# AlbrechtL/welle.io

Hardware: AMD Instinct MI355X
Metric: DAB Mode-I ensembles/s (x real-time) (higher is better)
Workload: dtype f32 (FFT/demap) + u16 (Viterbi metrics) + u8 (GF(256))

## Files before the change

welle.io_amd/capi.py:

```python
import ctypes as C
import os
import numpy as np

HERE = os.path.dirname(os.path.abspath(__file__))
DEFAULT_LIB = os.path.join(HERE, "libdabphy_hip.so")

T_U, T_S, FRAME_SYMS_LEN = 2048, 2552, 2048 + 75 * 2552
ABI_VERSION = 6


class Config(C.Structure):
    _fields_ = [("struct_size", C.c_uint32), ("n_ensembles", C.c_uint32), ("max_frames", C.c_uint32), ("device", C.c_int32),
                ("fft_placement", C.c_int32), ("disable_coarse", C.c_int32), ("want_constellation", C.c_int32),
                ("want_impulse_response", C.c_int32), ("demod_chunk", C.c_int32), ("freqsync_method", C.c_int32), ("pipeline_sync", C.c_int32), ("serial_sync", C.c_int32), ("no_batch_replay", C.c_int32), ("decode_shape", C.c_int32), ("sync_early", C.c_int32)]


class WidebandConfig(C.Structure):
    _fields_ = [("struct_size", C.c_uint32), ("decimation", C.c_uint32), ("n_taps", C.c_uint32), ("taps", C.POINTER(C.c_float)),
                ("offset_16khz", C.POINTER(C.c_int32)), ("format", C.c_int32)]


class ResamplerConfig(C.Structure):
    _fields_ = [("struct_size", C.c_uint32), ("interpolation", C.c_uint32), ("decimation", C.c_uint32), ("n_taps", C.c_uint32),
                ("taps", C.POINTER(C.c_float)), ("offset_16khz", C.POINTER(C.c_int32)), ("format", C.c_int32)]
# ... 248 lines not shown
        self._chk(self.lib.dabphy_time_viterbi(self.h, nbits, n_codewords, iters, C.byref(a), C.byref(b)))
        return a.value, b.value

    def time_copy(self, nbytes=2 << 30, blocks_per_cu=0, iters=5):
        a = C.c_float(0)
        self._chk(self.lib.dabphy_time_copy(self.h, C.c_uint64(nbytes), blocks_per_cu, iters, C.byref(a)))
        return a.value

    def traceback_split(self, on=True):
        self._chk(self.lib.dabphy_test_traceback_split(self.h, int(on)))

    def last_decode_plan(self):
        a = C.c_int32(0); b = C.c_int32(0)
        self._chk(self.lib.dabphy_last_decode_plan(self.h, C.byref(a), C.byref(b)))
        return a.value, b.value

    def time_fused_msc(self, iters=3):
        a = C.c_float(0)
        self._chk(self.lib.dabphy_time_fused_msc(self.h, iters, C.byref(a)))
        return a.value

    def reset(self):
        self._chk(self.lib.dabphy_reset(self.h))

    def stream_upload(self, iq, loop=False):
        iq = np.ascontiguousarray(iq, np.complex64).reshape(self.cfg.n_ensembles, -1)
        self._chk(self.lib.dabphy_stream_upload(self.h, _p(iq), C.c_uint64(iq.shape[1]), int(loop)))

    def stream_bind_device(self, dev_ptr, ring_samples, stride_samples, n_valid, loop=False):
        self._chk(self.lib.dabphy_stream_bind_device(self.h, C.c_void_p(dev_ptr), C.c_uint64(ring_samples), C.c_uint64(stride_samples),
# ... 352 lines not shown
```

welle.io_amd/csrc/dabphy_api.hip:

```cpp
#include "dabphy_internal.h"
#include <cstddef>

extern "C" {

uint32_t dabphy_abi_version(void) { return DABPHY_ABI_VERSION; }
size_t dabphy_struct_size(int32_t which)
{
    switch (which) {
        case DABPHY_STRUCT_CONFIG: return sizeof(dabphy_config);
        case DABPHY_STRUCT_FRAME_INFO: return sizeof(dabphy_frame_info);
        case DABPHY_STRUCT_SF_EVENT: return sizeof(dabphy_sf_event);
        case DABPHY_STRUCT_SUBCHANNEL: return sizeof(dabphy_subchannel);
        case DABPHY_STRUCT_PROTECTION: return sizeof(dabphy_protection);
        case DABPHY_STRUCT_TII_MEASUREMENT: return sizeof(dabphy_tii_measurement);
        case DABPHY_STRUCT_MSC_DESC: return sizeof(dabphy_msc_desc);
        case DABPHY_STRUCT_MP2_EVENT: return sizeof(dabphy_mp2_event);
        case DABPHY_STRUCT_AU_SERVICE: return sizeof(dabphy_au_service);
        case DABPHY_STRUCT_AU_DESC: return sizeof(dabphy_au_desc);
        case DABPHY_STRUCT_WIDEBAND_CONFIG: return sizeof(dabphy_wideband_config);
        case DABPHY_STRUCT_RESAMPLER_CONFIG: return sizeof(dabphy_resampler_config);
    }
    return 0;
}

// ... 22 lines not shown
    if (cfg_in->struct_size <= offsetof(dabphy_config, freqsync_method)) cfg_full.freqsync_method = 2;
    cfg_full.struct_size = (uint32_t)sizeof(dabphy_config);
    const dabphy_config* const cfg = &cfg_full;
    if (cfg->n_ensembles < 1 || cfg->max_frames < 1) return DABPHY_ERR_INVALID;
    if (cfg->max_frames > DABPHY_MAX_FRAMES || (uint64_t)cfg->n_ensembles * cfg->max_frames > DABPHY_MAX_ENSEMBLE_FRAMES) return DABPHY_ERR_INVALID;
    *out = nullptr;
    int ndev = 0;
    if (hipGetDeviceCount(&ndev) != hipSuccess || ndev <= 0 || cfg->device < 0 || cfg->device >= ndev) return DABPHY_ERR_NO_DEVICE;
    hipDeviceProp_t prop;
    if (hipGetDeviceProperties(&prop, cfg->device) != hipSuccess) return DABPHY_ERR_NO_DEVICE;
    if (strncmp(prop.gcnArchName, "gfx950", 6) != 0) return DABPHY_ERR_NO_DEVICE;
    if (hipSetDevice(cfg->device) != hipSuccess) return DABPHY_ERR_NO_DEVICE;
    dabphy_handle* h = new dabphy_handle();
    h->cfg = *cfg;
    h->subch_e.resize(cfg->n_ensembles); h->subch_next.resize(cfg->n_ensembles); h->where.resize(cfg->n_ensembles); h->kind_next.resize(cfg->n_ensembles);
    if (h->cfg.demod_chunk <= 0) h->cfg.demod_chunk = ((int64_t)h->cfg.n_ensembles * h->cfg.max_frames >= 1024) ? 25 : 15;
    if (h->cfg.demod_chunk > 75) h->cfg.demod_chunk = 75;
    snprintf(h->devname, sizeof h->devname, "%s (%s)", prop.name, prop.gcnArchName);
    int r = 0;
    auto fail = [&](int code) { dabphy_destroy(h); return code; };
    if (h->cfg.fft_placement < 0 || h->cfg.fft_placement > 2 || h->cfg.freqsync_method < 0 || h->cfg.freqsync_method > 2 || h->cfg.pipeline_sync < 0 || h->cfg.pipeline_sync > 3 || h->cfg.decode_shape < 0 || h->cfg.decode_shape > 3 || h->cfg.sync_early < 0 || h->cfg.sync_early > 3) return fail(DABPHY_ERR_INVALID);
    const HostTables& T = host_tables();
    if ((r = upload_const(h, &h->d_tw, T.tw))) return fail(r);
    if ((r = upload_const(h, &h->d_ref, T.ref))) return fail(r);
    if ((r = upload_const(h, &h->d_nco, T.nco))) return fail(r);
    if ((r = upload_const(h, &h->d_bin2soft, T.bin2soft))) return fail(r);
    if ((r = upload_const(h, &h->d_prbs_words, T.prbs_words))) return fail(r);
    dabphy_protection pf; protection_fic(&pf);
    if ((r = upload_const(h, &h->d_fic_map, depuncture_map(&pf)))) return fail(r);
    if ((r = upload_const(h, &h->d_osc_unsafe, T.osc_unsafe))) return fail(r);
    h->tab.tw = h->d_tw; h->tab.ref = h->d_ref; h->tab.nco = h->d_nco; h->tab.bin2soft = h->d_bin2soft; h->tab.prbs_bytes = nullptr;
    h->tab.osc_unsafe = h->d_osc_unsafe; h->tab.n_osc_unsafe = T.n_osc_unsafe;
    if ((r = device_block(h, &h->d_osc_stats, 2, true))) return fail(r);
    if ((r = device_block(h, &h->d_state, cfg->n_ensembles, true))) return fail(r);
    if ((r = device_block(h, &h->d_dec, cfg->n_ensembles, true))) return fail(r);
    {
        int n_placeholders = 5;
#ifdef DABPHY_EXPERIMENTS
        if (const char* e = getenv("DABPHY_STREAM_LAYOUT")) { h->stream_layout = atoi(e); n_placeholders = (h->stream_layout & 1) ? 5 : 0; }
#endif
        hipStream_t placeholder = nullptr;
        for (int i = 0; i < n_placeholders; i++) if ((r = new_stream(h, &placeholder, i == 1))) return fail(r);
    }
    if ((r = new_stream(h, &h->stream))) return fail(r);
    if ((r = new_stream(h, &h->sync_stream, true))) return fail(r);
    if ((r = new_stream(h, &h->aux_stream))) return fail(r);
    if ((r = new_stream(h, &h->copy_stream))) return fail(r);
    if (h->stream_layout & 2) h->fic_stream = h->aux_stream;
// ... 122 lines not shown
    if ((r = ensure(h, h->prs_mag, (size_t)n_frames * T_U * sizeof(float)))) return r;
    if ((r = ensure(h, h->snr, n_frames * sizeof(float)))) return r;
    if (constellation && (r = ensure(h, h->con, (size_t)n_frames * 1200 * sizeof(cf32)))) return r;
    std::vector<FrameDesc> d(n_frames);
    for (uint32_t f = 0; f < n_frames; f++) {
        memset(&d[f], 0, sizeof(FrameDesc));
        d[f].pos = (int64_t)(per * f); d[f].frame_no = f; d[f].valid = 1;
    }
    HIPCHK(h, hipMemcpyAsync(h->iq.p, frames, per * n_frames * sizeof(cf32), hipMemcpyHostToDevice, h->stream));
    HIPCHK(h, hipMemcpyAsync(h->desc.p, d.data(), n_frames * sizeof(FrameDesc), hipMemcpyHostToDevice, h->stream));
    DemodArgs a{};
    a.tab = h->tab; a.iq = h->iq.as<cf32>(); a.iq_stride = 0; a.ring = (int64_t)(per * n_frames);
    a.desc = h->desc.as<FrameDesc>(); a.n_frames = (int)n_frames; a.chunk_len = h->cfg.demod_chunk; a.mix = 0;
    a.soft = h->soft.as<int8_t>(); a.soft_ring = (int)n_frames;
    a.con = constellation ? h->con.as<cf32>() : nullptr; a.prs_mag = h->prs_mag.as<float>();
    launch_demod(a, 1, h->stream);
    SnrArgs s{}; s.state = h->d_dec; s.desc = a.desc; s.n_ens = 1; s.n_frames = (int)n_frames; s.prs_mag = a.prs_mag; s.snr_out = h->snr.as<float>();
    launch_snr(s, h->stream);
    HIPCHK(h, hipMemcpyAsync(soft, h->soft.p, (size_t)n_frames * SOFT_PER_FRAME, hipMemcpyDeviceToHost, h->stream));
    if (constellation) HIPCHK(h, hipMemcpyAsync(constellation, h->con.p, (size_t)n_frames * 1200 * sizeof(cf32), hipMemcpyDeviceToHost, h->stream));
    if (snr) HIPCHK(h, hipMemcpyAsync(snr, h->snr.p, n_frames * sizeof(float), hipMemcpyDeviceToHost, h->stream));
    return sync(h);
}

static int run_lin_decode(dabphy_handle* h, const int8_t* in, size_t in_stride, const map_t* d_map, int nbits, uint32_t n_cw,
                          int dedisperse, uint8_t* out)
{
    int r;
    if ((r = ensure(h, h->in8, in_stride * n_cw))) return r;
    VitClass c{};
    if ((r = prepare_class(h, c, nbits, (int)n_cw, dedisperse))) return r;
// ... 296 lines not shown
    for (uint32_t b = 0; b < n_ens; b++)
        for (uint32_t f = 0; f < n_frames; f++) {
            FrameDesc& x = d[(size_t)b * n_frames + f];
            memset(&x, 0, sizeof x);
            x.pos = (int64_t)(per * f); x.frame_no = f; x.valid = 1; x.f_prs = x.f_sym = f_hz; x.L0 = 12345; x.L1 = 54321;
            const HostTables& T = host_tables();
            for (int i = 0; i < T.n_osc_unsafe; i++) osc_hazard_entry(x.osc_hazard, T.osc_unsafe[i], x.start_index, x.L0, x.f_prs, x.L1, x.f_sym);
        }
    HIPCHK(h, hipMemcpyAsync(h->desc.p, d.data(), total * sizeof(FrameDesc), hipMemcpyHostToDevice, h->stream));
    DemodArgs a{};
    a.tab = h->tab; a.iq = h->iq.as<cf32>(); a.iq_stride = per * n_frames; a.ring = (int64_t)(per * n_frames);
    a.desc = h->desc.as<FrameDesc>(); a.n_frames = (int)n_frames; a.chunk_len = h->cfg.demod_chunk; a.mix = mix;
    a.soft = h->soft.as<int8_t>(); a.soft_ring = (int)n_frames; a.con = nullptr; a.prs_mag = nullptr;
    ScopedEvent e0, e1;
    HIPCHK(h, e0.create()); HIPCHK(h, e1.create());
    launch_demod(a, (int)n_ens, h->stream);
    HIPCHK(h, hipEventRecord(e0, h->stream));
    for (uint32_t i = 0; i < iters; i++) launch_demod(a, (int)n_ens, h->stream);
    HIPCHK(h, hipEventRecord(e1, h->stream));
    HIPCHK(h, hipEventSynchronize(e1));
    float t = 0; HIPCHK(h, hipEventElapsedTime(&t, e0, e1));
    *ms = t / iters;
    return sync(h);
}

int dabphy_time_copy(dabphy_handle* h, uint64_t bytes, uint32_t blocks_per_cu, uint32_t iters, float* gbytes_per_s)
{
    DeviceBind dev_(h);
    if (!h || !gbytes_per_s || bytes < 4096 || iters == 0) return DABPHY_ERR_INVALID;
    hipDeviceProp_t p;
    HIPCHK(h, hipGetDeviceProperties(&p, h->cfg.device));
    const int blocks = p.multiProcessorCount * (int)(blocks_per_cu ? blocks_per_cu : 4);
    DevBuf src, dst; int r;
// ... 43 lines not shown
        float a = 0, b = 0; HIPCHK(h, hipEventElapsedTime(&a, e0, e1)); HIPCHK(h, hipEventElapsedTime(&b, e1, e2));
        tg += a; tv += b;
    }
    *ms_gather = tg / iters; *ms_decode = tv / iters;
    return sync(h);
}

int dabphy_test_traceback_split(dabphy_handle* h, int32_t on)
{
    if (!h) return DABPHY_ERR_INVALID;
    h->tb_split = (on & 1) != 0;
    h->tb_no_walkers = (on & 2) == 0;
    return DABPHY_OK;
}

int dabphy_time_fused_msc(dabphy_handle* h, uint32_t iters, float* ms)
{
    DeviceBind dev_(h);
    if (!h || !ms || iters == 0) return DABPHY_ERR_INVALID;
    const auto& P = h->fplan;
    if (!P.valid || !P.launched || P.buf_gen != h->buf_gen || P.args.n_work == 0) { h->err = "no batch has been decoded by the fused kernel with the present buffers"; return DABPHY_ERR_STATE; }
    HIPCHK(h, hipDeviceSynchronize());
    ScopedEvent e0, e1;
    HIPCHK(h, e0.create()); HIPCHK(h, e1.create());
    const FusedSplit sp{h->tb_no_walkers ? nullptr : h->tb_stream, h->ev_tb_fork, h->ev_tb_join};
    auto again = [&]() { if (P.use_sp) launch_sp(P.args, P.sp_two, P.sp_variant, h->stream); else launch_viterbi_fused(P.args, P.variant, P.n_slots, h->stream, P.args.done ? &sp : nullptr); };
    again();
    HIPCHK(h, hipEventRecord(e0, h->stream));
    for (uint32_t i = 0; i < iters; i++) { again(); if (P.args.done) HIPCHK(h, hipStreamSynchronize(h->stream)); }
    HIPCHK(h, hipEventRecord(e1, h->stream));
// ... 8 lines not shown
```

welle.io_amd/csrc/dabphy_internal.h:

```cpp
#pragma once
#define DABPHY_BUILDING_LIBRARY
#include "../../include/dabphy.h"
#include "../../include/dabphy_test.h"
#include "dabphy_kernels.h"
#include "dabphy_host.h"
#include "osc_exact.h"
#include <string>
#include <vector>
#include <cstring>
#include <cstdio>
#include <cstdlib>
#include <cmath>
#include <algorithm>
#include <chrono>
#include <functional>
#include <numeric>

#define DABPHY_INTERNAL __attribute__((visibility("hidden")))

namespace dabphy {

inline bool debug_env(const char* name)
{
#ifdef DABPHY_EXPERIMENTS
// ... 20 lines not shown
constexpr int SF_BATCH_CLASSES = 256;
constexpr size_t SF_BATCH_BYTES = 3 * (SF_BATCH_CLASSES * sizeof(SfArgs) + (SF_BATCH_CLASSES + 1) * sizeof(int32_t) + 12);
struct HostTimeline { double acc[6] = {0, 0, 0, 0, 0, 0}; long n = 0; };
}
using namespace dabphy;

struct dabphy_handle {
    dabphy_config cfg{};
    hipStream_t stream = nullptr;
    std::string err;
    char devname[256] = {0};
    cf32 *d_tw = nullptr, *d_ref = nullptr, *d_nco = nullptr;
    int16_t* d_bin2soft = nullptr; uint32_t* d_prbs_words = nullptr; map_t* d_fic_map = nullptr;
    int32_t* d_osc_unsafe = nullptr; unsigned long long* d_osc_stats = nullptr;
    Tables tab{};
    DevBuf iq, soft, con, prs_mag, snr, desc, in8, map, vsym, vdec, vout, ok;
    DevBuf fsym, fdec;
    RxState* d_state = nullptr;
    DecState* d_dec = nullptr;
    std::vector<DevBuf> owned;
    std::vector<hipStream_t> streams; std::vector<hipEvent_t> events; std::vector<void*> pinned;

    struct MscClass {
        dabphy_protection prot{};
        std::vector<MscPair> pairs;
        std::vector<int32_t> subch_id, start_cu;
        bool cif0_pending = false;
        DevBuf map, pair_tab, tiles, out;
        DevBuf steps[FUSED_VARIANTS]; int n_windows[FUSED_VARIANTS] = {0, 0, 0};
        DevBuf sf_state;
// ... 261 lines not shown
    ta.tab = h->tab; ta.iq = iq; ta.iq_stride = iq_stride; ta.ring = ring; ta.desc = desc; ta.n_ens = (int)B; ta.n_frames = (int)F;
    ta.rot = h->tii_rot.as<cf32>(); ta.rank = h->tii_rank.as<int32_t>(); ta.pattern = h->tii_pat.as<uint8_t>();
    ta.abs_err = h->tii_err.as<float>(); ta.likely = h->tii_likely.as<int32_t>(); ta.state = h->tii_state.as<TiiSlot>();
    ta.events = h->tii_events.as<TiiEvent>(); ta.n_events = h->tii_nev.as<int32_t>(); ta.max_events = (int)h->tii_max_events;
    ta.overflow = tii_dropped(h);
    return ta;
}

inline int sync(dabphy_handle* h)
{
    HIPCHK(h, hipStreamSynchronize(h->stream));
    HIPCHK(h, hipGetLastError());
    return 0;
}

inline int prepare_class(dabphy_handle* h, VitClass& c, int nbits, int n_cw, int dedisperse)
{
    c.nbits = nbits; c.nsteps = nbits + 6; c.n_cw = n_cw; c.n_groups = (n_cw + 63) / 64; c.dedisperse = dedisperse; c.g_begin = 0; c.g_end = c.n_groups;
    const size_t cells = (size_t)c.n_groups * c.nsteps * 64;
    int r;
    if ((r = ensure(h, h->vsym, cells * sizeof(uint32_t)))) return r;
    if ((r = ensure(h, h->vdec, cells * sizeof(uint2)))) return r;
    if ((r = ensure(h, h->vout, (size_t)c.n_groups * 64 * (nbits / 8)))) return r;
    c.sym = h->vsym.as<uint32_t>(); c.dec = h->vdec.as<uint2>(); c.out = h->vout.as<uint8_t>();
    return 0;
}
inline VitArgs vit_args(const dabphy_handle* h, const VitClass& c) { VitArgs v{}; v.c = c; v.prbs_words = h->d_prbs_words; return v; }
inline FusedClass fic_fused_class(const dabphy_handle* h, uint8_t* out, int n_cw, int variant)
{
    FusedClass fc{}; fc.map = h->d_fic_map; fc.out = out; fc.nbits = 768; fc.nsteps = 774; fc.n_cw = n_cw; fc.n_pairs = 1; fc.kind = 1; fc.dedisperse = 1;
// ... 39 lines not shown
```

welle.io_amd/csrc/dabphy_kernels.h:

```cpp
#pragma once
#include "dabphy_common.h"

namespace dabphy {

struct RxState {
    int64_t pos;
    int64_t frame_no;
    int32_t local_phase;
    int32_t coarse;
    int32_t fine;
    int32_t synced;
    float s_level;
    int32_t lost;
    int32_t n_exact_sums;
    int32_t hist_count, hist_head;
    int32_t hist_dropped;
    int32_t n_relock_inexact;
    int32_t attempts;
    int32_t first_lock_attempts;
    int32_t n_wide_frames;
    int32_t n_chain_frames;
    int32_t calm_frames;
    int32_t acq_phase;
    int32_t acq_counter, acq_idx, acq_left;
// ... 45 lines not shown
    int skip_wide;
    int last_round;
};

struct DemodArgs {
    Tables tab;
    const cf32* iq; size_t iq_stride; int64_t ring;
    const FrameDesc* desc; int n_frames;
    int chunk_len;
    int mix;
    int8_t* soft; int soft_ring;
    size_t soft_ens_stride;
    cf32* con;
    float* prs_mag;
    unsigned long long* osc_stats;
    int frame_first, frame_count, chunk_count;
};

struct SnrArgs {
    DecState* state; const FrameDesc* desc; int n_ens, n_frames;
    const float* prs_mag; float* snr_out;
};

struct VitClass {
    int nbits;
    int nsteps;
    int n_cw;
    int n_groups;
    int g_begin, g_end;
    uint32_t* sym;
    uint2* dec;
// ... 241 lines not shown
struct AuSvc { int32_t n_superframes, n_aus, n_failed; uint32_t bytes; };
struct AuArgs {
    const SfEvent* events; const int32_t* n_events; int n_cif;
    const uint8_t* sf; int n_slots, sf_len;
    const int32_t* run;
    const MscPair* pairs; const int32_t* ens_base;
    int format;
    uint8_t* stage; uint64_t region0, reserve;
    AuSvc* svc; AuRec* aus; uint2* au_src; int au_cap;
};
void launch_au_pack(const AuArgs& a, int n_blocks, hipStream_t s);
void launch_superframe_bucket(const SfBatch& Bt, int bucket, int total_blocks, int n_cif, bool wide_pass, hipStream_t s);
void launch_rs_superframes(const RsArgs& a, hipStream_t s);
void launch_rs_msc(const RsMscArgs& a, hipStream_t s);

void launch_demod(const DemodArgs& a, int n_ens, hipStream_t s);
void launch_snr(const SnrArgs& a, hipStream_t s);
void launch_selftest_div127(unsigned long long* out, hipStream_t s);
void launch_selftest_unit_twiddle(unsigned long long* out, hipStream_t s);
void launch_viterbi(const VitArgs& a, hipStream_t s);
void launch_fic_gather(const FicGatherArgs& a, hipStream_t s);
void launch_msc_gather(const MscGatherArgs& a, hipStream_t s);
void launch_lin_gather(const LinGatherArgs& a, hipStream_t s);
void launch_fib_crc(const CrcArgs& a, hipStream_t s);
void launch_fic_ratio(const CrcArgs& a, hipStream_t s);
#ifdef SYNC_CHAIN_TS
void dump_chain_ts();
#endif
void launch_sync_find(const SyncArgs& a, hipStream_t s);
void launch_sync_wide(const SyncArgs& a, hipStream_t s, hipEvent_t front = nullptr);
void launch_sync_finish(const SyncArgs& a, hipStream_t s);
// ... 6 lines not shown
```

welle.io_amd/csrc/dabphy_process.hip:

```cpp
#include "dabphy_internal.h"

static inline double now_us() { return std::chrono::duration<double, std::micro>(std::chrono::steady_clock::now().time_since_epoch()).count(); }

struct Batch {
    uint32_t B = 0, F = 0;
    int cur = 0, depth = 0;
    int ring_frames = 0; size_t ens_stride = 0;
    FrameDesc* d_desc = nullptr;
    DemodArgs da{};
    VitClass fic{};
    double t0 = 0.0, t[6] = {0, 0, 0, 0, 0, 0};
};

static void tick(const dabphy_handle* h, Batch& b, int i) { if (h->tl_on) b.t[i] = now_us() - b.t0; }
static void mark(dabphy_handle* h, int stage, bool end, hipStream_t st = nullptr)
{
    if (!h->profiling) return;
    hipError_t e = hipEventRecord(end ? h->ev_end[stage] : h->ev_beg[stage], st ? st : h->stream); (void)e;
    h->ev_used[stage] = true;
}

static VitClass fic_class(const dabphy_handle* h, int n_cw)
{
    VitClass c{};
// ... 108 lines not shown
static int replay_fic_frames(dabphy_handle* h, const Batch& b)
{
    const uint32_t B = b.B, F = b.F;
    int r;
    SyncArgs sa = sync_args(h, b.cur, F, h->chain_valid[b.cur]);
    const VitClass c = fic_class(h, (int)(B * 4));
    CrcArgs k = crc_args(h, b);
    FicOneClass fic;
    if ((r = fic_one_prepare(h, fic, fic_gather_args(h, b, c), h->stream))) return r;
    for (uint32_t f = 0; f < F; f++) {
        sa.frame = (int)f;
        launch_sync_find(sa, h->stream);
        launch_sync_finish(sa, h->stream);
        DemodArgs d1 = b.da; d1.frame_first = (int)f; d1.frame_count = 1; d1.con = nullptr; d1.osc_stats = nullptr;
        d1.chunk_count = (3 + b.da.chunk_len - 1) / b.da.chunk_len;
        launch_demod(d1, (int)B, h->stream);
        k.frame_sel = (int)f + 1;
        fic_one_launch(h, fic, (int)f + 1, h->stream);
        launch_fib_crc(k, h->stream);
        CrcArgs kf = k; kf.frame_sel = 0; kf.frame_first = (int)f; kf.frame_count = 1;
        launch_fic_ratio(kf, h->stream);
    }
    return 0;
}

static int queue_next_chains(dabphy_handle* h, const Batch& b)
{
    int r;
    if (h->cfg.pipeline_sync != 2) HIPCHK(h, hipStreamWaitEvent(h->sync_stream, h->ev_chain_gate, 0));
    if (b.depth == 2 && h->ahead < 1 + b.depth && (r = sf_wait_for_pass(h, h->sync_stream))) return r;
    for (; h->ahead < 1 + b.depth; h->ahead++) if ((r = queue_chain(h, (b.cur + h->ahead) % dabphy_handle::N_DESC, b.F))) return r;
// ... 77 lines not shown
        g.map = cls.map.as<map_t>(); g.pairs = cls.pair_tab.as<MscPair>(); g.tiles = cls.tiles.as<int32_t>(); g.n_pairs = P; g.desc = b.d_desc; g.c = c;
        if (first_two) mark(h, dabphy_handle::ST_MSC_GATHER, false);
        launch_msc_gather(g, h->stream);
        launch_viterbi(vit_args(h, c), h->stream);
        first_two = false;
    }
    if (!first_two) mark(h, dabphy_handle::ST_MSC_GATHER, true);
    return 0;
}

static int decode_batch(dabphy_handle* h, Batch& b, const bool replay)
{
    int r;
    if (replay && (r = replay_fic_frames(h, b))) return r;
    mark(h, dabphy_handle::ST_DEMOD, false);
    launch_demod(b.da, (int)b.B, h->stream);
    tick(h, b, 2);
    mark(h, dabphy_handle::ST_DEMOD, true);
    if (!replay && (h->cfg.pipeline_sync == 1 || h->cfg.pipeline_sync == 3)) HIPCHK(h, hipEventRecord(h->ev_chain_gate, h->stream));
    if (!replay && b.depth == 2 && (r = sf_launch_waiting(h))) return r;
    const bool early = h->chain_early || (h->cfg.pipeline_sync != 2 && (h->cfg.sync_early == 0 || h->cfg.sync_early == 3 || (h->cfg.sync_early == 2 && h->drift_seen)));
    if (!replay && b.depth && early) {
        h->wide_front_recorded = false;
        if ((r = queue_next_chains(h, b))) return r;
        if (h->cfg.sync_early == 3 && h->wide_front_recorded) HIPCHK(h, hipStreamWaitEvent(h->stream, h->ev_wide_front, 0));
    }
    if (!replay && (r = sf_launch_waiting(h))) return r;
    if ((r = sf_wait_for_pass(h, h->stream))) return r;
    if ((r = queue_aux_work(h, b))) return r;
    for (auto& cls : h->classes) if (cls.cif0_pending) launch_pair_cif0(cls.pair_tab.as<MscPair>(), (int)cls.pairs.size(), b.d_desc, (int)b.F, h->stream);
    if ((r = launch_fused(h, b))) return r;
// ... 108 lines not shown
```

welle.io_amd/csrc/k_demod.hip:

```cpp
#include "fft2048.h"
#include "dabphy_kernels.h"
#include <dabphy_wave_ops.h>
#include "osc_exact.h"

namespace dabphy {

__device__ __forceinline__ int32_t mod_rate(int64_t x)
{
    int64_t r = x % INPUT_RATE;
    if (r < 0) r += INPUT_RATE;
    return (int32_t)r;
}

struct SymCursor { uint32_t a; int32_t ph; };
struct MixSteps { int32_t s128, sTS; uint32_t s256_bytes; int32_t f1; };

constexpr uint32_t NCO_BYTES = (uint32_t)INPUT_RATE * 8u;

struct OscChain { dc64 base, d128, d256, d512, d1024; };

__device__ __forceinline__ void osc_chain_steps(OscChain& k, int32_t f_hz)
{
    const dc64 a = osc_step(128, f_hz), b = osc_step(256, f_hz), b2 = osc_step(512, f_hz), b4 = osc_step(1024, f_hz);
    k.d128.re = uniform_f64(a.re); k.d128.im = uniform_f64(a.im);
// ... 251 lines not shown
                const int si = sidx_of(q);
                softbuf[si] = (fabsf(vr) < 2147483648.0f) ? (int8_t)(int)vr : (int8_t)0;
                softbuf[K_CARR + si] = (fabsf(vi) < 2147483648.0f) ? (int8_t)(int)vi : (int8_t)0;
            }
        }
        if (CON) {
#pragma unroll
            for (int q = 0; q < N_SLOTS; q++)
                if (sidx_of(q) % 96 == 0) con_frame[(s - 1) * 16 + sidx_of(q) / 96] = r1[q];
        }
    }
    __syncthreads();
    store_soft(s_end - 1);
    if (A.osc_stats && A.mix && t == 0) {
        atomicAdd(&A.osc_stats[0], (unsigned long long)((uint32_t)(s_end - s_begin) - n_checked));
        atomicAdd(&A.osc_stats[1], (unsigned long long)n_checked);
    }
}

__global__ void __launch_bounds__(64) k_snr_frames(SnrArgs A)
{
    const int lane = threadIdx.x, row = lane >> 4, l16 = lane & 15;
    const int n = A.n_ens * A.n_frames;
    int i = blockIdx.x * 4 + row;
    const bool live = i < n;
    if (!live) i = n - 1;
    const float* __restrict__ v = A.prs_mag + (size_t)i * T_U;
    constexpr int low = T_U / 2 - K_CARR / 2, high = low + K_CARR;
    constexpr int N1 = low - 20 - 70, N2 = 100, NS = K_CARR / 2;
    constexpr int B1 = (N1 + 15) / 16, B2 = (N2 + 15) / 16, BS = NS / 16;
// ... 75 lines not shown
        }
    }
    if (bad) atomicAdd(&out[0], bad);
    atomicAdd(&out[1], tried);
}
void launch_selftest_unit_twiddle(unsigned long long* out, hipStream_t s)
{
    hipLaunchKernelGGL(k_selftest_unit_twiddle, dim3(1u << 16), dim3(256), 0, s, out);
}

void launch_selftest_div127(unsigned long long* out, hipStream_t s)
{
    hipLaunchKernelGGL(k_selftest_div127, dim3(1u << 16), dim3(256), 0, s, out);
}

void launch_demod(const DemodArgs& a, int n_ens, hipStream_t s)
{
    int chunks = (75 + a.chunk_len - 1) / a.chunk_len;
    if (a.chunk_count > 0 && a.chunk_count < chunks) chunks = a.chunk_count;
    const int frames = a.frame_count > 0 ? a.frame_count : a.n_frames - a.frame_first;
    if (a.con) hipLaunchKernelGGL(k_demod<true>, dim3(chunks, frames, n_ens), dim3(FFT_THREADS), 0, s, a);
    else hipLaunchKernelGGL(k_demod<false>, dim3(chunks, frames, n_ens), dim3(FFT_THREADS), 0, s, a);
}

void launch_snr(const SnrArgs& a, hipStream_t s)
{
    hipLaunchKernelGGL(k_snr_frames, dim3((a.n_ens * a.n_frames + 3) / 4), dim3(64), 0, s, a);
    hipLaunchKernelGGL(k_snr, dim3((a.n_ens + 63) / 64), dim3(64), 0, s, a);
}

}
```

Before: 75900.

## Add persistent work-stealing demod kernel processing whole frames with cross-item DMA prefetch

Adds a persistent k_demod_frames kernel. It launches one workgroup per resident slot, and each workgroup pulls whole frames from a global atomic counter. Twiddle and bin2soft setup happens once per workgroup, and the LDS DMA for the next item's reference symbol is issued while the current symbol is transformed. The remainder frames are split into a few tail chunks to balance the end of the run. This path replaces the chunked grid launch whenever the default demod_chunk is used and there are enough frames. It removes the per-chunk reference-symbol recomputation and per-block setup, in exchange for atomic contention, a memset before each launch, and serialized whole-frame work per group.

Result: no change. 76240 (median of 4 runs) (+0.4%).

```diff
diff --git a/welle.io_amd/capi.py b/welle.io_amd/capi.py
--- a/welle.io_amd/capi.py
+++ b/welle.io_amd/capi.py
@@ -286,6 +286,25 @@
         a = C.c_int32(0); b = C.c_int32(0)
         self._chk(self.lib.dabphy_last_decode_plan(self.h, C.byref(a), C.byref(b)))
         return a.value, b.value
+
+    def demod_groups(self, groups):
+        self._chk(self.lib.dabphy_test_demod_groups(self.h, int(groups)))
+
+    def demod_path(self):
+        a = C.c_int32(0); b = C.c_uint64(0); c = C.c_uint64(0)
+        self._chk(self.lib.dabphy_test_demod_path(self.h, C.byref(a), C.byref(b), C.byref(c)))
+        return a.value, b.value, c.value
+
+    def demod_hazard(self, symbols=()):
+        m = (C.c_uint32 * 3)(0, 0, 0)
+        for s in symbols:
+            m[s // 32] |= 1 << (s % 32)
+        self._chk(self.lib.dabphy_test_demod_hazard(self.h, m))
+
+    def prs_magnitudes(self):
+        out = np.zeros((self.cfg.n_ensembles, self._last, 2048), np.float32)
+        self._chk(self.lib.dabphy_test_prs_magnitudes(self.h, _p(out)))
+        return out
 
     def time_fused_msc(self, iters=3):
         a = C.c_float(0)
diff --git a/welle.io_amd/csrc/dabphy_api.hip b/welle.io_amd/csrc/dabphy_api.hip
--- a/welle.io_amd/csrc/dabphy_api.hip
+++ b/welle.io_amd/csrc/dabphy_api.hip
@@ -60,6 +60,7 @@
     dabphy_handle* h = new dabphy_handle();
     h->cfg = *cfg;
     h->subch_e.resize(cfg->n_ensembles); h->subch_next.resize(cfg->n_ensembles); h->where.resize(cfg->n_ensembles); h->kind_next.resize(cfg->n_ensembles);
+    h->demod_frames_ok = h->cfg.demod_chunk <= 0;
     if (h->cfg.demod_chunk <= 0) h->cfg.demod_chunk = ((int64_t)h->cfg.n_ensembles * h->cfg.max_frames >= 1024) ? 25 : 15;
     if (h->cfg.demod_chunk > 75) h->cfg.demod_chunk = 75;
     snprintf(h->devname, sizeof h->devname, "%s (%s)", prop.name, prop.gcnArchName);
@@ -78,6 +79,7 @@
     h->tab.tw = h->d_tw; h->tab.ref = h->d_ref; h->tab.nco = h->d_nco; h->tab.bin2soft = h->d_bin2soft; h->tab.prbs_bytes = nullptr;
     h->tab.osc_unsafe = h->d_osc_unsafe; h->tab.n_osc_unsafe = T.n_osc_unsafe;
     if ((r = device_block(h, &h->d_osc_stats, 2, true))) return fail(r);
+    if ((r = device_block(h, &h->d_demod_next, 1, true))) return fail(r);
     if ((r = device_block(h, &h->d_state, cfg->n_ensembles, true))) return fail(r);
     if ((r = device_block(h, &h->d_dec, cfg->n_ensembles, true))) return fail(r);
     {
@@ -230,7 +232,7 @@
     a.desc = h->desc.as<FrameDesc>(); a.n_frames = (int)n_frames; a.chunk_len = h->cfg.demod_chunk; a.mix = 0;
     a.soft = h->soft.as<int8_t>(); a.soft_ring = (int)n_frames;
     a.con = constellation ? h->con.as<cf32>() : nullptr; a.prs_mag = h->prs_mag.as<float>();
-    launch_demod(a, 1, h->stream);
+    demod_launch(h, a, 1);
     SnrArgs s{}; s.state = h->d_dec; s.desc = a.desc; s.n_ens = 1; s.n_frames = (int)n_frames; s.prs_mag = a.prs_mag; s.snr_out = h->snr.as<float>();
     launch_snr(s, h->stream);
     HIPCHK(h, hipMemcpyAsync(soft, h->soft.p, (size_t)n_frames * SOFT_PER_FRAME, hipMemcpyDeviceToHost, h->stream));
@@ -557,9 +559,9 @@
     a.soft = h->soft.as<int8_t>(); a.soft_ring = (int)n_frames; a.con = nullptr; a.prs_mag = nullptr;
     ScopedEvent e0, e1;
     HIPCHK(h, e0.create()); HIPCHK(h, e1.create());
-    launch_demod(a, (int)n_ens, h->stream);
+    demod_launch(h, a, (int)n_ens);
     HIPCHK(h, hipEventRecord(e0, h->stream));
-    for (uint32_t i = 0; i < iters; i++) launch_demod(a, (int)n_ens, h->stream);
+    for (uint32_t i = 0; i < iters; i++) demod_launch(h, a, (int)n_ens);
     HIPCHK(h, hipEventRecord(e1, h->stream));
     HIPCHK(h, hipEventSynchronize(e1));
     float t = 0; HIPCHK(h, hipEventElapsedTime(&t, e0, e1));
@@ -633,6 +635,34 @@
     return DABPHY_OK;
 }
 
+int dabphy_test_demod_groups(dabphy_handle* h, int32_t groups)
+{
+    if (!h || groups < -1 || groups > 65536 || (groups != 0 && !h->demod_frames_ok)) return DABPHY_ERR_INVALID;
+    h->demod_groups = groups;
+    return DABPHY_OK;
+}
+int dabphy_test_demod_hazard(dabphy_handle* h, const uint32_t mask[3])
+{
+    if (!h) return DABPHY_ERR_INVALID;
+    for (int i = 0; i < 3; i++) h->demod_hazard_or[i] = mask ? mask[i] : 0u;
+    return DABPHY_OK;
+}
+int dabphy_test_prs_magnitudes(dabphy_handle* h, float* out)
+{
+    DeviceBind dev_(h);
+    if (!h || !out || !h->last_frames || !h->s_mag.p) return DABPHY_ERR_INVALID;
+    HIPCHK(h, hipMemcpyAsync(out, h->s_mag.p, (size_t)h->cfg.n_ensembles * h->last_frames * T_U * sizeof(float), hipMemcpyDeviceToHost, h->stream));
+    return sync(h);
+}
+int dabphy_test_demod_path(dabphy_handle* h, int32_t* last_groups, uint64_t* frame_launches, uint64_t* chunked_launches)
+{
+    if (!h) return DABPHY_ERR_INVALID;
+    if (last_groups) *last_groups = h->demod_last_groups;
+    if (frame_launches) *frame_launches = h->demod_frame_launches;
+    if (chunked_launches) *chunked_launches = h->demod_chunk_launches;
+    return DABPHY_OK;
+}
+
 int dabphy_time_fused_msc(dabphy_handle* h, uint32_t iters, float* ms)
 {
     DeviceBind dev_(h);
diff --git a/welle.io_amd/csrc/dabphy_internal.h b/welle.io_amd/csrc/dabphy_internal.h
--- a/welle.io_amd/csrc/dabphy_internal.h
+++ b/welle.io_amd/csrc/dabphy_internal.h
@@ -58,6 +58,9 @@
     int16_t* d_bin2soft = nullptr; uint32_t* d_prbs_words = nullptr; map_t* d_fic_map = nullptr;
     int32_t* d_osc_unsafe = nullptr; unsigned long long* d_osc_stats = nullptr;
     Tables tab{};
+    uint32_t* d_demod_next = nullptr; bool demod_frames_ok = false; int demod_groups = 0;
+    int demod_last_groups = 0; uint64_t demod_frame_launches = 0, demod_chunk_launches = 0;
+    uint32_t demod_hazard_or[3] = {0, 0, 0};
     DevBuf iq, soft, con, prs_mag, snr, desc, in8, map, vsym, vdec, vout, ok;
     DevBuf fsym, fdec;
     RxState* d_state = nullptr;
@@ -349,6 +352,14 @@
     return 0;
 }
 
+inline void demod_launch(dabphy_handle* h, DemodArgs a, int n_ens)
+{
+    a.next = h->demod_frames_ok ? h->d_demod_next : nullptr; a.groups = h->demod_groups;
+    for (int i = 0; i < 3; i++) a.hazard_or[i] = h->demod_hazard_or[i];
+    h->demod_last_groups = launch_demod(a, n_ens, h->stream);
+    (h->demod_last_groups ? h->demod_frame_launches : h->demod_chunk_launches) += 1;
+}
+
 inline int prepare_class(dabphy_handle* h, VitClass& c, int nbits, int n_cw, int dedisperse)
 {
     c.nbits = nbits; c.nsteps = nbits + 6; c.n_cw = n_cw; c.n_groups = (n_cw + 63) / 64; c.dedisperse = dedisperse; c.g_begin = 0; c.g_end = c.n_groups;
diff --git a/welle.io_amd/csrc/dabphy_kernels.h b/welle.io_amd/csrc/dabphy_kernels.h
--- a/welle.io_amd/csrc/dabphy_kernels.h
+++ b/welle.io_amd/csrc/dabphy_kernels.h
@@ -83,7 +83,12 @@
     cf32* con;
     float* prs_mag;
     unsigned long long* osc_stats;
+    uint32_t hazard_or[3];
     int frame_first, frame_count, chunk_count;
+    uint32_t* next;
+    int groups;
+    uint32_t n_items, n_whole;
+    int tail_chunks, tail_len;
 };
 
 struct SnrArgs {
@@ -355,7 +360,8 @@
 void launch_rs_superframes(const RsArgs& a, hipStream_t s);
 void launch_rs_msc(const RsMscArgs& a, hipStream_t s);
 
-void launch_demod(const DemodArgs& a, int n_ens, hipStream_t s);
+int launch_demod(const DemodArgs& a, int n_ens, hipStream_t s);
+int demod_frame_groups(const DemodArgs& a, int n_ens);
 void launch_snr(const SnrArgs& a, hipStream_t s);
 void launch_selftest_div127(unsigned long long* out, hipStream_t s);
 void launch_selftest_unit_twiddle(unsigned long long* out, hipStream_t s);
diff --git a/welle.io_amd/csrc/dabphy_process.hip b/welle.io_amd/csrc/dabphy_process.hip
--- a/welle.io_amd/csrc/dabphy_process.hip
+++ b/welle.io_amd/csrc/dabphy_process.hip
@@ -146,7 +146,7 @@
         launch_sync_finish(sa, h->stream);
         DemodArgs d1 = b.da; d1.frame_first = (int)f; d1.frame_count = 1; d1.con = nullptr; d1.osc_stats = nullptr;
         d1.chunk_count = (3 + b.da.chunk_len - 1) / b.da.chunk_len;
-        launch_demod(d1, (int)B, h->stream);
+        demod_launch(h, d1, (int)B);
         k.frame_sel = (int)f + 1;
         fic_one_launch(h, fic, (int)f + 1, h->stream);
         launch_fib_crc(k, h->stream);
@@ -254,7 +254,7 @@
     int r;
     if (replay && (r = replay_fic_frames(h, b))) return r;
     mark(h, dabphy_handle::ST_DEMOD, false);
-    launch_demod(b.da, (int)b.B, h->stream);
+    demod_launch(h, b.da, (int)b.B);
     tick(h, b, 2);
     mark(h, dabphy_handle::ST_DEMOD, true);
     if (!replay && (h->cfg.pipeline_sync == 1 || h->cfg.pipeline_sync == 3)) HIPCHK(h, hipEventRecord(h->ev_chain_gate, h->stream));
diff --git a/welle.io_amd/csrc/k_demod.hip b/welle.io_amd/csrc/k_demod.hip
--- a/welle.io_amd/csrc/k_demod.hip
+++ b/welle.io_amd/csrc/k_demod.hip
@@ -289,6 +289,266 @@
     store_soft(s_end - 1);
     if (A.osc_stats && A.mix && t == 0) {
         atomicAdd(&A.osc_stats[0], (unsigned long long)((uint32_t)(s_end - s_begin) - n_checked));
+        atomicAdd(&A.osc_stats[1], (unsigned long long)n_checked);
+    }
+}
+
+
+__shared__ __attribute__((aligned(16))) cf32 demod_tile[FFT_INPLACE_TILE];
+__shared__ __attribute__((aligned(16))) cf32 demod_twB[FFT_TWB_ENTRIES];
+__shared__ __attribute__((aligned(16))) int8_t demod_softbuf[SOFT_PER_SYM];
+__shared__ __attribute__((aligned(16))) dc64 demod_symstep[L_SYM];
+__shared__ uint16_t demod_sidx[N_SLOTS * FFT_THREADS];
+struct DemodStage { const cf32* iq; uint32_t a0; bool ok; };
+
+__device__ __forceinline__ void demod_group_setup(FftTwiddles& w, const DemodArgs& A, int t)
+{
+    fft_load_twiddles(w, A.tab.tw, demod_twB, t);
+#pragma unroll
+    for (int q = 0; q < N_SLOTS; q++) {
+        const int j = q >= 6 ? q + 4 : (q == 0 && t == 0) ? 6 : q;
+        demod_sidx[q * FFT_THREADS + t] = (uint16_t)A.tab.bin2soft[t + 128 * j];
+    }
+}
+
+__device__ __forceinline__ void demod_dma_issue(const DemodStage& g, int t)
+{
+    const int lane = t & 63, wvu = uniform_i32(t >> 6);
+    const char* p = reinterpret_cast<const char*>(g.iq + g.a0 + 1024 * wvu) + 16 * lane;
+    cf32* l = demod_tile + 4 * FFT_RAW_PITCH * wvu;
+#pragma unroll
+    for (int r = 0; r < 4; r++) { lds_dma16<0>(p + 2048 * r, l + FFT_RAW_PITCH * r); lds_dma16<1024>(p + 2048 * r, l + FFT_RAW_PITCH * r); }
+}
+
+__device__ __forceinline__ int32_t demod_symbol_offset(int32_t start_index, int s) { return s == 0 ? start_index : start_index + T_U + (s - 1) * T_S + T_G; }
+
+__device__ __forceinline__ void demod_store_soft(int8_t* dst8, int t)
+{
+    const uint2* src = reinterpret_cast<const uint2*>(demod_softbuf);
+    uint2* dst = reinterpret_cast<uint2*>(dst8);
+#pragma unroll
+    for (int i = 0; i < 3; i++) dst[t + 128 * i] = src[t + 128 * i];
+}
+
+__device__ __forceinline__ void demod_open_symbol(bool staged, int8_t* soft_pend, int t)
+{
+    if (staged) lds_dma_wait();
+    __syncthreads();
+    if (soft_pend) demod_store_soft(soft_pend, t);
+}
+
+template <typename Hook>
+__device__ __forceinline__ void demod_transform(cf32 (&v)[16], const FftTwiddles& w, int t, bool staged, const cf32* __restrict__ iq,
+                                                uint32_t ring, const SymCursor& c, const OscChain& osc, const cf32* __restrict__ nco,
+                                                const MixSteps& ms, int mix, bool checked, Hook after_c_reads)
+{
+#pragma unroll
+    for (int h = 0; h < 2; h++) {
+        cf32 x[8];
+        if (staged) fft_raw_half(x, demod_tile, h, t); else load_raw_half(x, iq, ring, c, h);
+        mix_half(x, c, osc, nco, ms, h, mix, checked);
+        fft_round_a_inplace<false>(x, h, demod_tile, w, t);
+    }
+    fft_rounds_bc_split<false>(v, demod_tile, w, t, after_c_reads);
+}
+
+template <bool CON>
+__device__ __forceinline__ void demod_demap(const cf32 (&v)[16], cf32 (&prev)[N_SLOTS], cf32* con_sym, int t)
+{
+    int8_t* const softbuf = demod_softbuf;
+    auto sidx_of = [&](int q) { return (int)demod_sidx[q * FFT_THREADS + t]; };
+#ifdef DEMOD_EXP_NODEMAP
+    {
+        uint32_t* sb = reinterpret_cast<uint32_t*>(softbuf);
+#pragma unroll
+        for (int q = 0; q < 6; q++) {
+            uint32_t acc = __float_as_uint(v[q].re) ^ __float_as_uint(v[q].im) ^ __float_as_uint(v[q + 6].re) ^ __float_as_uint(v[q + 6].im);
+            if (q < 4) acc ^= __float_as_uint(v[q + 12].re) ^ __float_as_uint(v[q + 12].im);
+            sb[t + 128 * q] = acc;
+        }
+        return;
+    }
+#endif
+    cf32 r1[N_SLOTS]; float l1[N_SLOTS];
+    {
+        cf32 cs[N_SLOTS]; carrier_slots(cs, v, t);
+#pragma unroll
+        for (int q = 0; q < N_SLOTS; q++) {
+            r1[q] = pk_cmulc(cs[q], prev[q]);
+            l1[q] = l1norm(r1[q]);
+            prev[q] = cs[q];
+        }
+    }
+    float lo = l1[0], hi = l1[0];
+#pragma unroll
+    for (int q = 1; q < N_SLOTS; q++) { lo = fminf(lo, l1[q]); hi = fmaxf(hi, l1[q]); }
+    if (wave_all(lo >= DIV127_LO && hi <= DIV127_HI)) {
+#pragma unroll
+        for (int q = 0; q < N_SLOTS; q++) {
+            const float ab1 = div127_fast<DIV127_VARIANT>(l1[q]);
+            const float vr = (-r1[q].re) * ab1, vi = (-r1[q].im) * ab1;
+            const int si = sidx_of(q);
+            softbuf[si] = (int8_t)cvt_i32_trunc(vr);
+            softbuf[K_CARR + si] = (int8_t)cvt_i32_trunc(vi);
+        }
+    } else {
+#pragma unroll
+        for (int q = 0; q < N_SLOTS; q++) {
+            const float ab1 = 127.0f / l1[q];
+            const float vr = (-r1[q].re) * ab1, vi = (-r1[q].im) * ab1;
+            const int si = sidx_of(q);
+            softbuf[si] = (fabsf(vr) < 2147483648.0f) ? (int8_t)(int)vr : (int8_t)0;
+            softbuf[K_CARR + si] = (fabsf(vi) < 2147483648.0f) ? (int8_t)(int)vi : (int8_t)0;
+        }
+    }
+    if (CON) {
+#pragma unroll
+        for (int q = 0; q < N_SLOTS; q++)
+            if (sidx_of(q) % 96 == 0) con_sym[sidx_of(q) / 96] = r1[q];
+    }
+}
+
+template <bool CON, typename Next>
+__device__ __forceinline__ void demod_item(const DemodArgs& A, const FftTwiddles& w, int t, int b, int f, int s_begin, int s_end,
+                                           DemodStage& st, int8_t*& soft_pend, uint32_t& n_checked, Next next)
+{
+    const FrameDesc d = A.desc[(size_t)b * A.n_frames + f];
+    const cf32* __restrict__ iq = A.iq + (size_t)b * A.iq_stride;
+    const cf32* __restrict__ nco = A.tab.nco;
+    const uint32_t ring = (uint32_t)A.ring;
+    const int32_t J0 = d.start_index + T_U;
+    auto cursor_at = [&](int32_t off) {
+        SymCursor c;
+        c.a = (uint32_t)((d.pos + off + t) % A.ring);
+        if (off < J0) c.ph = mod_rate((int64_t)d.L0 - (int64_t)(off + t + 1) * d.f_prs);
+        else c.ph = mod_rate((int64_t)d.L1 - (int64_t)(off - J0 + t + 1) * d.f_sym);
+        return c;
+    };
+    auto steps_for = [&](int32_t fhz) { MixSteps m; m.s128 = mod_rate(128LL * fhz); m.s256_bytes = 8u * (uint32_t)mod_rate(256LL * fhz); m.sTS = mod_rate((int64_t)T_S * fhz); m.f1 = mod_rate((int64_t)fhz); return m; };
+    const uint32_t hz0 = d.osc_hazard[0] | A.hazard_or[0], hz1 = d.osc_hazard[1] | A.hazard_or[1], hz2 = d.osc_hazard[2] | A.hazard_or[2];
+#ifdef DEMOD_FORCE_CHECKED
+    auto hazard_bit = [&](int) { return DEMOD_FORCE_CHECKED != 0; };
+#else
+    auto hazard_bit = [&](int sym) { return (((sym < 32 ? hz0 : sym < 64 ? hz1 : hz2) >> (sym & 31)) & 1u) != 0; };
+#endif
+    auto dma_ok = [&](uint32_t a0) { return a0 + (uint32_t)T_U <= ring; };
+
+    cf32 prev[N_SLOTS], v[16];
+    OscChain osc{};
+    const int sref = s_begin - 1;
+    uint32_t sym0 = (uint32_t)((d.pos + demod_symbol_offset(d.start_index, s_begin)) % A.ring);
+    DemodStage cur_st; cur_st.iq = iq; cur_st.a0 = sym0; cur_st.ok = dma_ok(sym0);
+    {
+        const SymCursor c = cursor_at(demod_symbol_offset(d.start_index, sref));
+        const MixSteps msr = steps_for(sref == 0 ? d.f_prs : d.f_sym);
+        if (A.mix) { osc_chain_steps(osc, sref == 0 ? d.f_prs : d.f_sym); osc.base = osc_exp(c.ph); }
+        demod_open_symbol(st.ok, soft_pend, t);
+        demod_transform(v, w, t, st.ok, iq, ring, c, osc, nco, msr, A.mix, hazard_bit(sref), [&]() { if (cur_st.ok) demod_dma_issue(cur_st, t); });
+        if (sref == 0 && A.prs_mag) {
+            float* pm = A.prs_mag + ((size_t)b * A.n_frames + f) * T_U;
+#pragma unroll
+            for (int j = 0; j < 16; j++) pm[t + 128 * j] = hypotf_exact(v[j].re, v[j].im);
+        }
+        carrier_slots(prev, v, t);
+    }
+    const size_t slot = (size_t)((d.frame_no) % A.soft_ring);
+    int8_t* soft_frame = A.soft + (size_t)b * (A.soft_ens_stride ? A.soft_ens_stride : (size_t)A.soft_ring * SOFT_PER_FRAME) + slot * SOFT_PER_FRAME;
+    cf32* con_frame = CON ? A.con + ((size_t)b * A.n_frames + f) * 1200 : nullptr;
+
+    SymCursor cur = cursor_at(demod_symbol_offset(d.start_index, s_begin));
+    const MixSteps ms = steps_for(d.f_sym);
+    dc64 base0{};
+    if (A.mix) {
+        if (sref == 0 && d.f_prs != d.f_sym) osc_chain_steps(osc, d.f_sym);
+        base0 = osc_exp(cur.ph); osc.base = base0;
+        if (t < s_end - s_begin) demod_symstep[t] = osc_step((int64_t)t * T_S, d.f_sym);
+    }
+    soft_pend = nullptr;
+    for (int s = s_begin; s < s_end; s++) {
+        const bool checked = hazard_bit(s);
+        n_checked += checked ? 1u : 0u;
+        demod_open_symbol(cur_st.ok, soft_pend, t);
+        DemodStage nx;
+        if (s + 1 < s_end) { nx.iq = iq; nx.a0 = cur_st.a0 + T_S; if (nx.a0 >= ring) nx.a0 -= ring; nx.ok = dma_ok(nx.a0); }
+        else nx = next();
+        demod_transform(v, w, t, cur_st.ok, iq, ring, cur, osc, nco, ms, A.mix, checked, [&]() { if (nx.ok) demod_dma_issue(nx, t); });
+        cur_st = nx;
+        cur.a += T_S; if (cur.a >= ring) cur.a -= ring;
+        cur.ph -= ms.sTS; if (cur.ph < 0) cur.ph += INPUT_RATE;
+        if (A.mix && s + 1 < s_end) osc.base = osc_mul(base0, demod_symstep[s + 1 - s_begin]);
+        demod_demap<CON>(v, prev, CON ? con_frame + (s - 1) * 16 : nullptr, t);
+        soft_pend = soft_frame + (size_t)(s - 1) * SOFT_PER_SYM;
+    }
+    st = cur_st;
+}
+
+struct DemodWork { int b, f, s_begin, s_end; };
+__device__ __forceinline__ DemodWork demod_work(const DemodArgs& A, uint32_t item)
+{
+    DemodWork k;
+    uint32_t fi = item;
+    k.s_begin = 1; k.s_end = L_SYM;
+    if (item >= A.n_whole) {
+        const uint32_t j = item - A.n_whole;
+        fi = A.n_whole + j / (uint32_t)A.tail_chunks;
+        k.s_begin = 1 + (int)(j % (uint32_t)A.tail_chunks) * A.tail_len;
+        k.s_end = k.s_begin + A.tail_len; if (k.s_end > L_SYM) k.s_end = L_SYM;
+    }
+    k.b = (int)(fi / (uint32_t)A.frame_count); k.f = A.frame_first + (int)(fi % (uint32_t)A.frame_count);
+    return k;
+}
+__device__ __forceinline__ uint32_t demod_pull(const DemodArgs& A, int lane)
+{
+    for (;;) {
+        uint32_t item = 0;
+        if (lane == 0) item = atomicAdd(A.next, 1u);
+        item = (uint32_t)uniform_i32(__shfl((int)item, 0));
+        if (item >= A.n_items) return A.n_items;
+        const DemodWork k = demod_work(A, item);
+        if (A.desc[(size_t)k.b * A.n_frames + k.f].valid == 1) return item;
+    }
+}
+__device__ __forceinline__ DemodStage demod_reference_stage(const DemodArgs& A, uint32_t item)
+{
+    DemodStage g{nullptr, 0u, false};
+    if (item >= A.n_items) return g;
+    const DemodWork k = demod_work(A, item);
+    const FrameDesc& d = A.desc[(size_t)k.b * A.n_frames + k.f];
+    g.iq = A.iq + (size_t)k.b * A.iq_stride;
+    g.a0 = (uint32_t)((d.pos + demod_symbol_offset(d.start_index, k.s_begin - 1)) % A.ring);
+    g.ok = g.a0 + (uint32_t)T_U <= (uint32_t)A.ring;
+    return g;
+}
+
+template <bool CON>
+__global__ void __launch_bounds__(FFT_THREADS, DEMOD_WAVES) k_demod_frames(DemodArgs A)
+{
+    __shared__ uint32_t s_item[2];
+    const int t = threadIdx.x, lane = t & 63, wvu = uniform_i32(t >> 6);
+    FftTwiddles w; demod_group_setup(w, A, t);
+    if (wvu == 0) s_item[0] = demod_pull(A, lane);
+    __syncthreads();
+    uint32_t item = (uint32_t)uniform_i32((int)s_item[0]);
+    int par = 1;
+    DemodStage st = demod_reference_stage(A, item);
+    if (st.ok) demod_dma_issue(st, t);
+    int8_t* soft_pend = nullptr;
+    uint32_t n_checked = 0, n_symbols = 0;
+    while (item < A.n_items) {
+        if (wvu == 0) s_item[par] = demod_pull(A, lane);
+        const DemodWork k = demod_work(A, item);
+        uint32_t item_next = A.n_items;
+        demod_item<CON>(A, w, t, k.b, k.f, k.s_begin, k.s_end, st, soft_pend, n_checked, [&]() {
+            item_next = (uint32_t)uniform_i32((int)s_item[par]);
+            return demod_reference_stage(A, item_next);
+        });
+        n_symbols += (uint32_t)(k.s_end - k.s_begin);
+        item = item_next; par ^= 1;
+    }
+    __syncthreads();
+    if (soft_pend) demod_store_soft(soft_pend, t);
+    if (A.osc_stats && A.mix && t == 0 && n_symbols) {
+        atomicAdd(&A.osc_stats[0], (unsigned long long)(n_symbols - n_checked));
         atomicAdd(&A.osc_stats[1], (unsigned long long)n_checked);
     }
 }
@@ -394,13 +654,54 @@
     hipLaunchKernelGGL(k_selftest_div127, dim3(1u << 16), dim3(256), 0, s, out);
 }
 
-void launch_demod(const DemodArgs& a, int n_ens, hipStream_t s)
-{
+static int demod_resident_groups(bool con)
+{
+#ifdef HIPEMU
+    (void)con;
+    return 256 * 4 * DEMOD_WAVES / (FFT_THREADS / 64);
+#else
+    static int n[2] = {0, 0};
+    if (!n[con]) {
+        int dev = 0, per_cu = 0; hipDeviceProp_t p;
+        const hipError_t e = con ? hipOccupancyMaxActiveBlocksPerMultiprocessor(&per_cu, k_demod_frames<true>, FFT_THREADS, 0)
+                                 : hipOccupancyMaxActiveBlocksPerMultiprocessor(&per_cu, k_demod_frames<false>, FFT_THREADS, 0);
+        if (e == hipSuccess && per_cu > 0 && hipGetDevice(&dev) == hipSuccess && hipGetDeviceProperties(&p, dev) == hipSuccess) n[con] = per_cu * p.multiProcessorCount;
+        else { (void)hipGetLastError(); return 0; }
+    }
+    return n[con];
+#endif
+}
+int demod_frame_groups(const DemodArgs& a, int n_ens)
+{
+    if (!a.next || a.chunk_count > 0 || a.groups == 0) return 0;
+    if (a.groups > 0) return a.groups;
+    const int frames = a.frame_count > 0 ? a.frame_count : a.n_frames - a.frame_first;
+    const int resident = demod_resident_groups(a.con != nullptr);
+    return (resident > 0 && (int64_t)frames * n_ens >= resident) ? resident : 0;
+}
+int launch_demod(const DemodArgs& a, int n_ens, hipStream_t s)
+{
+    const int frames = a.frame_count > 0 ? a.frame_count : a.n_frames - a.frame_first;
+    if (frames <= 0 || n_ens <= 0) return 0;
+    const int groups = demod_frame_groups(a, n_ens);
+    if (groups > 0) {
+        DemodArgs k = a;
+        k.frame_count = frames;
+        const uint32_t total = (uint32_t)frames * (uint32_t)n_ens, rest = total % (uint32_t)groups;
+        k.n_whole = total - rest;
+        k.tail_chunks = rest ? std::max(1, std::min(5, groups / (int)rest)) : 1;
+        k.tail_len = (75 + k.tail_chunks - 1) / k.tail_chunks;
+        k.n_items = k.n_whole + rest * (uint32_t)k.tail_chunks;
+        hipError_t e = hipMemsetAsync(k.next, 0, sizeof(uint32_t), s); (void)e;
+        if (k.con) hipLaunchKernelGGL(k_demod_frames<true>, dim3(groups), dim3(FFT_THREADS), 0, s, k);
+        else hipLaunchKernelGGL(k_demod_frames<false>, dim3(groups), dim3(FFT_THREADS), 0, s, k);
+        return groups;
+    }
     int chunks = (75 + a.chunk_len - 1) / a.chunk_len;
     if (a.chunk_count > 0 && a.chunk_count < chunks) chunks = a.chunk_count;
-    const int frames = a.frame_count > 0 ? a.frame_count : a.n_frames - a.frame_first;
     if (a.con) hipLaunchKernelGGL(k_demod<true>, dim3(chunks, frames, n_ens), dim3(FFT_THREADS), 0, s, a);
     else hipLaunchKernelGGL(k_demod<false>, dim3(chunks, frames, n_ens), dim3(FFT_THREADS), 0, s, a);
+    return 0;
 }
 
 void launch_snr(const SnrArgs& a, hipStream_t s)
```
